# pashtari/factorizer

Hardware: AMD Instinct MI355X
Metric: volumes/sec fwd+bwd, Swin Factorizer 128^3 (higher is better)
Workload: dtype f32

## Files before the change

### factorizer_amd/_native.py

```python
from __future__ import annotations

import ctypes
import os
import threading

import torch

_HERE = os.path.dirname(os.path.abspath(__file__))
LIB_PATH = os.environ.get("FZ_LIB_PATH") or os.path.join(_HERE, "libfactorizer_hip.so")

FZ_OK = 0
FZ_E_UNSUPPORTED = -2
ABI_VERSION = 7
SOLVER_ID = {"mu": 0, "hals": 1, "cd": 2, "smu": 3}
STORE_F32, STORE_BF16 = 0, 1
PRODUCTS_DEFAULT, PRODUCTS_SPLIT_BF16, PRODUCTS_FP32_MFMA = 0, 1, 2
_products = threading.local()


def products() -> int:
    return getattr(_products, "value", PRODUCTS_DEFAULT)


class use_products:
# ... 132 lines not shown
                ("Di", _i), ("Hi", _i), ("Wi", _i), ("w", _vp), ("w_t", _i), ("ldw", _i), ("M", _i), ("K", _i),
                ("bias", _vp), ("ln", _i), ("ln_g", _vp), ("ln_b", _vp), ("ln_eps", _f), ("stats_out", _vp),
                ("bact", _i), ("bmul", _vp), ("bmul_kind", _i), ("eact", _i), ("res", _vp), ("emul", _vp), ("emul_kind", _i), ("y", _vp),
                ("Ncol", _i64), ("Ho", _i), ("Wo", _i), ("B", _i), ("loader", _i), ("epilogue", _i), ("lnb_x", _vp), ("lnb_stats", _vp), ("lnb_g", _vp),
                ("lnb_gadd", _vp), ("lnb_part", _vp), ("act_dtype", _i), ("products", _i), ("tune", _i)]


class MlpDesc(_c.Structure):
    _fields_ = [("mode", _i), ("inp", _vp), ("w1", _vp), ("w2", _vp), ("b1", _vp), ("b2", _vp), ("ln_g", _vp),
                ("ln_b", _vp), ("ln_eps", _f), ("stats", _vp), ("z1", _vp), ("gz1", _vp), ("x1", _vp), ("out", _vp),
                ("part", _vp), ("B", _i), ("C", _i), ("H", _i), ("V", _i64), ("act_dtype", _i), ("wpart", _vp),
                ("gw1", _vp), ("gb1", _vp), ("gw2", _vp), ("gb2", _vp), ("gln", _vp), ("glp", _vp), ("products", _i),
                ("pre_in", _vp), ("pre_w", _vp), ("pre_b", _vp), ("pre_res", _vp), ("pre_out", _vp),
                ("post_w", _vp), ("post_b", _vp), ("post_out", _vp), ("post_m", _i)]


class MlpDropout(_c.Structure):
    _fields_ = [("m0", _vp), ("m1", _vp), ("m2", _vp), ("s0", _f), ("s1", _f), ("s2", _f)]


class BlockPrologue(_c.Structure):
    _fields_ = [("ln_g", _vp), ("ln_b", _vp), ("ln_eps", _f), ("w", _vp), ("t", _vp), ("stats", _vp)]


class GemmDwDesc(_c.Structure):
    _fields_ = [("g", _vp), ("q", _vp), ("w", _vp), ("ln", _i), ("stats", _vp), ("ln_g", _vp), ("ln_b", _vp), ("gadd", _vp),
                ("y", _vp), ("gln", _vp), ("wpart", _vp), ("gw", _vp), ("gb", _vp), ("B", _i), ("C", _i), ("V", _i64),
                ("act_dtype", _i), ("ldgw", _i), ("ldw", _i), ("drop_m", _vp), ("drop_s", _f)]


class WgradDesc(_c.Structure):
    _fields_ = [("p", _vp), ("M", _i), ("pmul", _vp), ("pmul_kind", _i), ("q", _vp * 4), ("nsrc", _i),
                ("src_mode", _i), ("c0", _i), ("Cin", _i), ("K", _i), ("Vq", _i64), ("D", _i), ("H", _i),
                ("W", _i), ("N", _i64), ("Ho", _i), ("Wo", _i), ("stats", _vp), ("qact", _i), ("ln_g", _vp),
                ("ln_b", _vp), ("gw", _vp), ("gbias", _vp), ("accumulate", _i), ("B", _i), ("loader", _i),
                ("act_dtype", _i), ("products", _i)]


class VolGeom(_c.Structure):
    _fields_ = [("nd", _i), ("size", _i * 3), ("start", _i * 3), ("end", _i * 3), ("pad", _i * 3), ("out", _i * 3)]


class RespaceGeom(_c.Structure):
    _fields_ = [("nd", _i), ("src_size", _i * 3), ("src_axis", _i * 3), ("flip", _i * 3), ("res_size", _i * 3), ("pad", _i * 3),
                ("out", _i * 3), ("orig_size", _i * 3), ("box_start", _i * 3), ("scale", _c.c_double * 3),
                ("inv_scale", _c.c_double * 3)]


_SIGS.update({
    "fz_gcorr_supported": ([_i] * 5, _i),
    "fz_gcorr": ([_vp] * 5 + [_i] * 11 + [_f, _vp], _i),
    "fz_gcorr_wgrad_workspace_bytes": ([_i] * 10, _i64),
    "fz_gcorr_wgrad": ([_vp] * 4 + [_i] * 11 + [_vp], _i),
    "fz_gcorr_act": ([_vp] * 5 + [_i] * 11 + [_f, _i, _vp], _i),
    "fz_gcorr_wgrad_act": ([_vp] * 4 + [_i] * 12 + [_vp], _i),
    "fz_gcorr_mu_bwd": ([_vp] * 8 + [_i] * 11 + [_f, _i, _vp], _i),
    "fz_gnmf_supported": ([_i, _i64, _i, _i, _i], _i),
    "fz_gnmf_workspace_bytes": ([_i64, _i, _i64, _i, _i, _i], _i64),
    "fz_gnmf_launches": ([_i, _i, _i], _i),
    "fz_gnmf_fwd": ([_vp] * 6 + [_i64, _i, _i64, _i, _i, _i, _f, _vp, _vp], _i),
    "fz_gnmf_bwd": ([_vp] * 7 + [_i64, _i, _i64, _i, _i, _i, _i, _f, _vp, _vp], _i),
    "fz_nmf_cf_supported": ([_i] * 11, _i),
    "fz_nmf_cf_fwd": ([_vp] * 4 + [_i] * 5 + [_c.POINTER(_i)] + [_i] * 5 + [_f, _i, _vp], _i),
    "fz_nmf_cf_bwd": ([_vp] * 5 + [_i] * 5 + [_c.POINTER(_i)] + [_i] * 7 + [_f, _i, _vp], _i),
    "fz_nmf_cf_factors_supported": ([_i] * 12 + [_c.POINTER(_i)], _i),
    "fz_nmf_cf_fwd_store_factors": ([_vp] * 5 + [_i] * 5 + [_c.POINTER(_i)] + [_i] * 3 + [_f, _i, _vp], _i),
    "fz_nmf_cf_fwd_from_factors": ([_vp] * 6 + [_i] * 5 + [_c.POINTER(_i)] * 2 + [_i] * 4 + [_f, _i, _vp], _i),
    "fz_nmf_cf_bwd_factors_supported": ([_i] * 14 + [_c.POINTER(_i)], _i),
    "fz_nmf_cf_bwd_store_factors": ([_vp] * 5 + [_i] * 5 + [_c.POINTER(_i)] + [_i] * 3 + [_f, _i, _vp], _i),
    "fz_nmf_cf_bwd_from_factors": ([_vp] * 6 + [_i] * 5 + [_c.POINTER(_i)] * 2 + [_i] * 3 + [_f, _i, _vp], _i),
    "fz_nmf_pcf_supported": ([_i] * 11, _i),
    "fz_nmf_pcf_fwd": ([_vp] * 4 + [_i] * 8 + [_c.POINTER(_i)] + [_i] * 5 + [_f, _i, _vp], _i),
    "fz_nmf_pcf_bwd": ([_vp] * 5 + [_i] * 8 + [_c.POINTER(_i)] + [_i] * 7 + [_f, _i, _vp], _i),
    "fz_nmf_pcf_bwd_prefers_separate": ([_i] * 4, _i),
    "fz_act_add": ([_vp, _vp, _i64, _i, _vp], _i),
    "fz_mlp_pre_supported": ([_i, _i, _i64, _i], _i),
    "fz_mlp_drop_supported": ([_i, _i, _i64, _i], _i),
    "fz_mlp_chain_drop": ([_c.POINTER(MlpDesc), _c.POINTER(MlpDropout), _vp], _i),
    "fz_conv3_prologue_supported": ([_i] * 4, _i),
    "fz_conv3_fwd2": ([_vp] * 4 + [_i] * 8 + [_c.POINTER(BlockPrologue), _vp], _i),
    "fz_upcat2": ([_vp, _vp, _vp, _i, _vp, _vp, _vp] + [_i] * 7 + [_c.POINTER(BlockPrologue), _vp], _i),
    "fz_gemm": ([_c.POINTER(GemmDesc), _vp], _i),
    "fz_gemm_bx_enable": ([_i], _i),
    "fz_gemm_lnbwd_partials": ([_c.POINTER(GemmDesc)], _i64),
    "fz_reduce_rows": ([_vp, _i64, _i, _vp, _vp, _vp], _i),
    "fz_adamw_step": ([_vp, _vp, _vp, _vp, _i64, _f, _f, _f, _f, _f, _i, _f, _vp], _i),
    "fz_sw_gather": ([_vp, _vp] + [_i] * 10 + [_vp], _i),
    "fz_sw_accumulate": ([_vp] * 6 + [_f] + [_i] * 10 + [_vp], _i),
    "fz_sw_finalize": ([_vp, _vp, _i, _i64, _vp], _i),
    "fz_sw_gather2": ([_vp, _vp] + [_i] * 11 + [_vp], _i),
    "fz_sw_accumulate2": ([_vp] * 6 + [_f] + [_i] * 11 + [_vp], _i),
    "fz_sw_finalize2": ([_vp, _vp, _vp, _i, _i64, _i, _vp], _i),
    "fz_mlp_supported": ([_i, _i, _i64], _i),
    "fz_mlp_partials": ([_i, _i64], _i64),
    "fz_mlp_wgrad_rows": ([_i, _i64], _i),
    "fz_gemm_dw_rows": ([_i, _i64], _i),
    "fz_gemm_dw_workspace_bytes": ([_i, _i64], _i64),
    "fz_gemm_dw": ([_c.POINTER(GemmDwDesc), _vp], _i),
    "fz_mlp_wgrad_workspace_bytes": ([_i, _i64], _i64),
    "fz_mlp_chain": ([_c.POINTER(MlpDesc), _vp], _i),
    "fz_head_bwd_rows": ([], _i),
    "fz_head_bwd_workspace_bytes": ([], _i64),
    "fz_head_bwd": ([_vp, _vp, _vp, _vp, _vp, _i, _i, _i, _i64, _i, _vp], _i),
    "fz_head_fwd": ([_vp, _vp, _vp, _vp, _i, _i, _i, _i64, _i, _vp], _i),
    "fz_upcat_supported": ([_i] * 5, _i),
    "fz_upcat_compose": ([_vp, _vp, _i, _vp, _vp, _vp, _vp, _vp, _i, _i, _i, _vp], _i),
    "fz_upcat_wgrads": ([_vp, _vp, _vp, _i, _vp, _vp, _vp, _vp, _i, _vp, _i, _i, _i, _vp], _i),
    "fz_upcat": ([_vp, _vp, _vp, _i, _vp, _vp, _vp] + [_i] * 7 + [_vp], _i),
    "fz_upcat_bwd_supported": ([_i] * 6, _i),
    "fz_upcat_bwd_workspace_bytes": ([_i] * 4, _i64),
    "fz_upcat_bwd": ([_vp, _vp, _vp, _vp, _i, _vp, _vp, _vp, _vp, _vp, _i, _vp, _vp] + [_i] * 7 + [_vp], _i),
    "fz_wgrad": ([_c.POINTER(WgradDesc), _vp, _vp], _i),
    "fz_wgrad_group": ([_c.POINTER(_c.POINTER(WgradDesc)), _c.POINTER(_vp), _i, _vp], _i),
    "fz_wgrad_workspace_bytes": ([_c.POINTER(WgradDesc)], _i64),
    "fz_conv3_fwd": ([_vp] * 4 + [_i] * 8 + [_vp], _i),
    "fz_conv3_wgrad_chunks": ([_i] * 4, _i),
    "fz_conv3_wgrad_partials": ([_vp] * 4 + [_i] * 8 + [_vp], _i),
    "fz_chunk_reduce": ([_vp, _i, _i64, _vp, _i, _vp], _i),
    "fz_chunk_reduce_ld": ([_vp, _i, _i64, _i64, _vp, _i, _vp], _i),
    "fz_finish_defer": ([_i], _i),
    "fz_finish_pending": ([], _i),
    "fz_finish_flush": ([_vp], _i),
    "fz_finish_flush_all": ([_vp], _i),
    "fz_dice_bce_chunks": ([_i64], _i),
    "fz_dice_bce_sums": ([_vp, _vp, _vp, _i, _i64, _vp], _i),
    "fz_dice_bce_grad": ([_vp, _vp, _vp, _vp, _i, _i64, _f, _f, _vp, _vp], _i),
    "fz_dice_ce_sums": ([_vp, _vp, _vp, _i, _i, _i64, _vp], _i),
    "fz_dice_ce_grad": ([_vp, _vp, _vp, _vp, _i, _i, _i64, _f, _f, _vp, _vp], _i),
    "fz_dice_ce_finish": ([_vp, _i, _i, _i64, _f, _vp, _vp, _vp], _i),
    "fz_rowsum_chunks": ([_i64], _i),
    "fz_rowsum": ([_vp, _vp, _vp, _i, _i, _i64, _i, _vp], _i),
    "fz_ln_fwd": ([_vp] * 5 + [_i, _i, _i64, _f, _i, _vp], _i),
    "fz_ln_bwd": ([_vp] * 8 + [_i, _i, _i64, _i, _vp], _i),
    "fz_ln_bwd_workspace_bytes": ([_i], _i64),
    "fz_ln_bwd_workspace_bytes2": ([_i, _i, _i64], _i64),
    "fz_dropout_bits_words": ([_i, _i, _i64], _i64),
    "fz_dropout_keep_bits": ([_vp, _i, _i, _i, _i64, _f, _vp, _vp], _i),
    "fz_dropout_apply": ([_i, _vp, _f, _vp, _vp, _vp, _i, _i, _i64, _i, _vp], _i),
    "fz_seg_counts_chunks": ([_i64], _i),
    "fz_seg_counts_workspace_bytes": ([_i, _i64], _i64),
    "fz_seg_counts": ([_vp, _i, _vp, _i, _f, _vp, _vp, _vp, _i, _i64, _vp], _i),
    "fz_mask_edges": ([_vp, _vp, _vp, _i, _i, _i, _i, _i, _vp], _i),
    "fz_edge_min_dist2_splits": ([_i64, _i64], _i),
    "fz_edge_min_dist2_workspace_bytes": ([_i64, _i64], _i64),
    "fz_edge_min_dist2": ([_vp, _i64, _vp, _i64, _f, _f, _f, _vp, _vp, _vp], _i),
    "fz_aug_record_floats": ([], _i),
    "fz_aug_resample": ([_vp, _vp, _i, _i, _vp, _vp, _i, _vp, _vp, _vp] + [_i] * 6 + [_vp], _i),
    "fz_aug_smooth": ([_vp, _vp, _i, _i, _vp, _vp] + [_i] * 6 + [_vp], _i),
    "fz_aug_noise_field": ([_vp, _vp, _i, _i, _i64, _vp], _i),
    "fz_aug_source_words": ([], _i),
    "fz_aug_crop_resample": ([_vp, _vp, _i, _i, _vp, _i, _vp, _vp, _vp] + [_i] * 6 + [_vp], _i),
    "fz_vol_kind_ok": ([_i, _i], _i),
    "fz_vol_bbox": ([_vp, _i, _i, _i, _i, _i, _i, _vp, _vp], _i),
    "fz_vol_workspace_bytes": ([_i, _c.POINTER(VolGeom)], _i64),
    "fz_vol_stats": ([_vp, _i, _i, _c.POINTER(VolGeom), _i, _i, _vp, _vp], _i),
    "fz_vol_write": ([_vp, _i, _vp, _i, _i, _vp, _i, _i, _c.POINTER(_i), _c.POINTER(_i), _i, _vp, _c.POINTER(VolGeom), _i, _i,
                      _vp, _vp, _vp, _vp], _i),
    "fz_vol_restore": ([_c.POINTER(_vp), _i, _i, _i, _c.POINTER(VolGeom), _f, _c.POINTER(_c.c_ubyte), _vp, _vp], _i),
    "fz_vol_respace": ([_vp, _i, _vp, _i, _vp, _i, _vp, _c.POINTER(RespaceGeom), _i, _vp], _i),
    "fz_vol_unspace": ([_c.POINTER(_vp), _i, _i, _i, _c.POINTER(RespaceGeom), _i, _i, _f, _vp, _vp], _i),
})
SEG_F32, SEG_BF16, SEG_U8 = 0, 1, 2
VOL_F32, VOL_BF16, VOL_U8, VOL_I16 = 0, 1, 2, 3
VOL_IMAGE_IN, VOL_IMAGE_OUT, VOL_LABEL_IN, VOL_LOGITS = 0, 1, 2, 3
RESPACE_BILINEAR, RESPACE_NEAREST = 0, 1
DROP_RES, DROP_GELU, DROP_GELU_BWD = 0, 1, 2
# ... 1 lines not shown
```

### factorizer_amd/build.py

```python
from __future__ import annotations

import concurrent.futures as cf
import os
import shutil
import subprocess
import sys

HERE = os.path.dirname(os.path.abspath(__file__))
CSRC = os.path.join(HERE, "csrc")
OBJ = os.path.join(HERE, "csrc", "build")
LIB = os.path.join(HERE, "libfactorizer_hip.so")
ARCH = "gfx950"
FLAGS = ["--offload-arch=" + ARCH, "-O3", "-std=c++17", "-fPIC", "-fno-gpu-rdc", "-Wno-comment",
         "-ffp-contract=fast"]
_SLP_ON = {"gemm_bx.hip"}


def flags_of(src: str) -> list:
    return FLAGS if src in _SLP_ON else [*FLAGS, "-fno-slp-vectorize"]


def _hipcc() -> str:
    exe = shutil.which("hipcc") or "/opt/rocm/bin/hipcc"
    if not os.path.exists(exe):
        raise RuntimeError("hipcc not found: cannot build libfactorizer_hip.so")
    return exe


def sources():
    return sorted(f for f in os.listdir(CSRC) if f.endswith(".hip"))


def _newest(suffixes) -> float:
    m = 0.0
    for root in (CSRC, os.path.join(os.path.dirname(HERE), "include")):
        for f in os.listdir(root):
            if f.endswith(suffixes):
                m = max(m, os.path.getmtime(os.path.join(root, f)))
    return m


def _stale_flags() -> bool:
    for src in sources():
        stamp = os.path.join(OBJ, src[:-4] + ".o.flags")
        if not os.path.exists(stamp) or open(stamp).read() != " ".join(flags_of(src)):
            return True
    return False


def needs_build() -> bool:
    return not os.path.exists(LIB) or os.path.getmtime(LIB) < _newest((".h", ".inc", ".hip")) or _stale_flags()


def _compile(src: str) -> str:
    obj = os.path.join(OBJ, src[:-4] + ".o")
    flags = flags_of(src)
    stamp, want = obj + ".flags", " ".join(flags)
    fresh = os.path.exists(stamp) and open(stamp).read() == want
    if fresh and os.path.exists(obj) and os.path.getmtime(obj) >= max(os.path.getmtime(os.path.join(CSRC, src)), _newest((".h", ".inc"))):
        return obj
    cmd = [_hipcc(), *flags, "-c", os.path.join(CSRC, src), "-o", obj]
    r = subprocess.run(cmd, capture_output=True, text=True)
    if r.returncode != 0:
        raise RuntimeError(f"hipcc failed on {src}:\n{r.stderr[-4000:]}")
    with open(stamp, "w") as f:
        f.write(want)
    return obj


def build(force: bool = False, verbose: bool = True, jobs: int | None = None) -> str:
    if not force and not needs_build():
        return LIB
    os.makedirs(OBJ, exist_ok=True)
    srcs = sources()
    jobs = jobs or min(len(srcs), int(os.environ.get("MAX_JOBS") or 0) or min(os.cpu_count() or 4, 16))
    if verbose:
        print(f"[factorizer_amd] hipcc {ARCH}: {len(srcs)} translation units, {jobs} jobs", flush=True)
    with cf.ThreadPoolExecutor(jobs) as ex:
        objs = list(ex.map(_compile, srcs))
    tmp = LIB + ".tmp"
    r = subprocess.run([_hipcc(), "--offload-arch=" + ARCH, "-shared", "-fPIC", "-o", tmp, *objs],
                       capture_output=True, text=True)
    if r.returncode != 0:
        raise RuntimeError("link failed:\n" + r.stderr[-4000:])
    os.replace(tmp, LIB)
    if verbose:
        print(f"[factorizer_amd] built {LIB}", flush=True)
    return LIB


if __name__ == "__main__":
    build(force="--force" in sys.argv)
```

### factorizer_amd/csrc/gemm_bx.h

```cpp
#pragma once
#include "gemm_common.h"

namespace fz {

typedef __bf16 bx8 __attribute__((ext_vector_type(8)));
typedef __bf16 bx2 __attribute__((ext_vector_type(2)));
typedef float fx2 __attribute__((ext_vector_type(2)));

enum { BXPRO_NONE = 0, BXPRO_LN = 1, BXPRO_GELU = 2, BXPRO_BMUL = 3 };

template <int NT>
__device__ __forceinline__ void bx_split(const float (&x)[8], bx8 (&t)[NT]) {
#pragma unroll
  for (int i = 0; i < 8; i += 2) {
    fx2 v = {x[i], x[i + 1]};
    const bx2 a = __builtin_convertvector(v, bx2);
    t[0][i] = a[0]; t[0][i + 1] = a[1];
    if constexpr (NT >= 2) {
      v = v - __builtin_convertvector(a, fx2);
      const bx2 b = __builtin_convertvector(v, bx2);
      t[1][i] = b[0]; t[1][i + 1] = b[1];
      if constexpr (NT >= 3) {
        v = v - __builtin_convertvector(b, fx2);
        const bx2 c = __builtin_convertvector(v, bx2);
// ... 111 lines not shown
      constexpr int RBT = NACC == 4 ? 4 : (NACC == 2 ? 8 : 16);
#pragma unroll
      for (int r0 = 0; r0 < 16; r0 += RBT) {
      float ev[RBT][NACC], rv[RBT][NACC];
      if (p.emul != nullptr) {
#pragma unroll
        for (int rr = 0; rr < RBT; ++rr) uload<NACC>(p.emul + (urow + ((r0 + rr) & 3) + 8 * ((r0 + rr) >> 2)) * p.Ncol, yoff, ev[rr]);
      }
      if (p.res != nullptr) {
#pragma unroll
        for (int rr = 0; rr < RBT; ++rr) uload<NACC>(p.res + (urow + ((r0 + rr) & 3) + 8 * ((r0 + rr) >> 2)) * p.Ncol, yoff, rv[rr]);
      }
#pragma unroll
      for (int rr = 0; rr < RBT; ++rr) {
        const int r = r0 + rr;
        const int rl = (r & 3) + 8 * (r >> 2) + 4 * h;
        float add = sBias[mb * 32 + rl];
        float v[NACC];
        if (LN) {
          const float sw = sW[mb * 32 + rl];
          add += tW[mb * 32 + rl];
#pragma unroll
          for (int q = 0; q < NACC; ++q) v[q] = rstd[q] * (acc[mb][q][r] - mu_d[q] * sw) + add;
        } else {
#pragma unroll
          for (int q = 0; q < NACC; ++q) v[q] = acc[mb][q][r] + add;
        }
        if (p.eact) {
#pragma unroll
          for (int q = 0; q < NACC; ++q) v[q] = act_f(p.eact, v[q]);
        }
        if (p.emul != nullptr) {
#pragma unroll
          for (int q = 0; q < NACC; ++q) v[q] *= act_grad_f(p.emul_kind, ev[rr][q]);
        }
        if (p.res != nullptr) {
#pragma unroll
          for (int q = 0; q < NACC; ++q) v[q] += rv[rr][q];
        }
        AT* yp = reinterpret_cast<AT*>(reinterpret_cast<char*>(p.y + (urow + (r & 3) + 8 * (r >> 2)) * p.Ncol) + yoff);
        vstore<NACC>(yp, v);
      }
      }
    }
  } else {
    const int Wf = 2 * p.Wo, Hf = 2 * p.Ho;
    const int64_t Vf = 8 * p.Ncol;
    const int Mo = p.M >> 3;
    const int wo = (int)(col_off % p.Wo);
    const int64_t t2 = col_off / p.Wo;
    const int ho = (int)(t2 % p.Ho);
    const int dz = (int)(t2 / p.Ho);
    const unsigned foff = (unsigned)((((int64_t)(2 * dz + h) * Hf + 2 * ho) * Wf + 2 * wo) * ES);
#pragma unroll
    for (int mb = 0; mb < MB; ++mb) {
      const int64_t uo = (int64_t)b * Mo + ((m0 + mb * 32) >> 3);
      float rv[8][2 * NACC];
      if (p.res != nullptr) {
#pragma unroll
        for (int rp = 0; rp < 8; ++rp)
          uload<2 * NACC>(p.res + (uo + (rp >> 1)) * Vf + (int64_t)(rp & 1) * Wf, foff, rv[rp]);
      }
#pragma unroll
      for (int rp = 0; rp < 8; ++rp) {
        const int r0 = 2 * rp;
        const float bs = sBias[mb * 32 + 8 * (rp >> 1)];
        float v[2 * NACC];
#pragma unroll
        for (int q = 0; q < NACC; ++q) { v[2 * q] = acc[mb][q][r0] + bs; v[2 * q + 1] = acc[mb][q][r0 + 1] + bs; }
        if (p.res != nullptr) {
#pragma unroll
          for (int i = 0; i < 2 * NACC; ++i) v[i] += rv[rp][i];
        }
        AT* yp = reinterpret_cast<AT*>(reinterpret_cast<char*>(p.y + (uo + (rp >> 1)) * Vf + (int64_t)(rp & 1) * Wf) + foff);
        vstore<2 * NACC>(yp, v);
      }
    }
  }
}

template <typename AT>
int gemm_bxk_launch(const GemmArgsT<AT>& a, int loader, int epilogue, int pro, int nacc, int mb, fz_stream_t stream);

}
```

### factorizer_amd/csrc/gemm_bx.hip

```cpp
#include "gemm_bx.h"

namespace fz {

template <int MB, int NACC, int LOADER, int EPI, int PRO, int RD, bool WT, typename AT>
__global__ __launch_bounds__(256, 2) void gemm_bx_kernel(GemmArgsT<AT> p) {
  constexpr int NTA = BxTerms<AT>::A, NTB = bx_terms_b<AT>(PRO);
  constexpr int TN = 32 * NACC;
  constexpr bool S2D = LOADER == LOAD_S2D;
  static_assert(!S2D || NACC == 2, "space-to-depth loader: two coarse voxels per lane");
  constexpr int NL = S2D ? 4 : NACC;
  constexpr int SPG = S2D ? 4 : 8;
  constexpr int ES = (int)sizeof(AT);
  constexpr bool LN = PRO == BXPRO_LN, GATE = PRO == BXPRO_BMUL;
  constexpr int CH = 4;
  static_assert(CH % RD == 0, "ring slots must be static inside a chunk");
  constexpr int kItemHalfs = 8;
  constexpr int kBufItems = CH * MB * NTA * 64;
  constexpr int IPT = CH * MB * 64 / 256;
  __shared__ __attribute__((aligned(16))) __bf16 As[2 * kBufItems * kItemHalfs];
  __shared__ float sW[32 * MB];
  __shared__ float tW[32 * MB];
  __shared__ float sBias[32 * MB];
  __shared__ float sRed[LN ? 2 * 256 : 1];

// ... 211 lines not shown
  for (int e = 0; e < NACC; ++e) { mu_d[e] = 0.f; rstd[e] = 1.f; }
  if (LN) {
    sRed[threadIdx.x] = sWp;
    sRed[256 + threadIdx.x] = tWp;
    __syncthreads();
    if (threadIdx.x < 32 * MB) {
      const int mb = threadIdx.x >> 5, i = threadIdx.x & 31;
      float a = 0.f, c = 0.f;
      for (int w = mb; w < 4; w += MB)
        for (int hh = 0; hh < 2; ++hh) { a += sRed[64 * w + 32 * hh + i]; c += sRed[256 + 64 * w + 32 * hh + i]; }
      sW[threadIdx.x] = a;
      tW[threadIdx.x] = c;
    }
#pragma unroll
    for (int e = 0; e < NACC; ++e) {
      const float t1 = s1[e] + __shfl_xor(s1[e], 32, 64);
      const float t2 = s2[e] + __shfl_xor(s2[e], 32, 64);
      const float inv = 1.0f / (float)p.Cin;
      const float md = t1 * inv;
      float var = t2 * inv - md * md;
      var = var > 0.f ? var : 0.f;
      mu_d[e] = md;
      rstd[e] = 1.0f / sqrtf(var + p.ln_eps);
    }
    if (p.stats_out != nullptr && by == 0 && h == 0 && col_ok) {
      float mean[NACC];
#pragma unroll
      for (int e = 0; e < NACC; ++e) mean[e] = shift[e] + mu_d[e];
      float* so = p.stats_out + (int64_t)b * 2 * p.Vin;
      vstore<NACC>(so + col_off, mean);
      vstore<NACC>(so + p.Vin + col_off, rstd);
    }
    __syncthreads();
  }
  if (!col_ok) return;
  bx_epilogue<MB, NACC, EPI, S2D, LN, AT>(p, acc, b, m0, n0, j, h, col_off, sBias, sW, tW, rstd, mu_d);
}

template <typename AT>
bool gemm_bx_ok(const GemmArgsT<AT>& a, int loader, int epilogue, int pro, int nacc) {
  if (a.K % 32 != 0 || a.M % 32 != 0) return false;
  if (loader == LOAD_PLAIN && (a.c0 % 16 != 0 || a.Cin != a.K)) return false;
  if (loader == LOAD_S2D && (8 * a.Cin != a.K || pro != BXPRO_NONE || epilogue != EPI_PLAIN || (a.Wo & 1))) return false;
  if (epilogue == EPI_D2S && (pro != BXPRO_NONE || (nacc >= 2 && (a.Wo % nacc) != 0))) return false;
  if (a.Ncol % nacc != 0 || a.Vin % nacc != 0) return false;
  if (!a.w_t && ((a.ldw & 3) != 0 || (reinterpret_cast<uintptr_t>(a.w) & 15) != 0)) return false;
  if (pro == BXPRO_LN && ((reinterpret_cast<uintptr_t>(a.ln_g) & 15) != 0 || (reinterpret_cast<uintptr_t>(a.ln_b) & 15) != 0)) return false;
  const int64_t es = (int64_t)sizeof(AT);
  if ((8 * a.Vin + a.Vin) * es >= ((int64_t)1 << 31)) return false;
  if (((int64_t)a.M * a.ldw + 8 * a.ldw) * 4 >= ((int64_t)1 << 31)) return false;
  if ((4 * a.Ncol + a.Ncol) * es * 8 >= ((int64_t)1 << 31)) return false;
  return true;
}

template <typename AT>
int gemm_bx_launch(const GemmArgsT<AT>& a0, int loader, int epilogue, int pro, fz_stream_t stream) {
  GemmArgsT<AT> a = a0;
  hipStream_t st = (hipStream_t)stream;
  const int mblocks = (a.M + 31) / 32;
  int nacc, mb;
  {
    int ks = (a.Ncol * a.B <= 4096 || (a.Ncol * a.B <= 8192 && a.K >= 512)) ? 1 : 0;
    int kn = 2, km = mblocks >= 2 ? 2 : 1;
    auto wgs = [&](int na, int mbb) { return ((a.Ncol + 32 * na - 1) / (32 * na)) * a.B * ((mblocks + mbb - 1) / mbb); };
    if (wgs(kn, km) < 512 && km == 2) km = 1;
    if (wgs(kn, km) < 512 && loader != LOAD_S2D) kn = 1;
    if (a.tune >= 100) {
      ks = a.tune / 100 == 2;
      if (ks) { kn = (a.tune / 10) % 10; km = a.tune % 10; if (km > mblocks) km = 1; if (loader == LOAD_S2D) kn = 2; if (kn < 1 || kn > 2) kn = 2; if (km < 1 || km > 2) km = 1; }
    }
    if (ks) {
      const int rc = gemm_bxk_launch<AT>(a, loader, epilogue, pro, kn, km, stream);
      if (rc != FZ_E_UNSUPPORTED) return rc;
    }
  }
  if (loader == LOAD_S2D) {
    nacc = 2;
    mb = mblocks >= 2 ? 2 : 1;
  } else {
    nacc = 4; mb = mblocks >= 2 ? 2 : 1;
    auto wgs = [&](int na, int mbb) { return ((a.Ncol + 128 * na - 1) / (128 * na)) * a.B * ((mblocks + mbb - 1) / mbb); };
    if (wgs(nacc, mb) < 512) nacc = 2;
    if (wgs(nacc, mb) < 512 && mb == 2) mb = 1;
    if (a.tune / 100 == 1) { nacc = (a.tune / 10) % 10; mb = a.tune % 10; if (mb > mblocks || mb < 1) mb = 1; }
    if (nacc != 2 && nacc != 4) nacc = 2;
    if (pro == BXPRO_LN || pro == BXPRO_BMUL) nacc = 2;
  }
  if (mblocks % mb != 0) mb = 1;
  if (!gemm_bx_ok(a, loader, epilogue, pro, nacc)) return FZ_E_UNSUPPORTED;
  const int TN = 32 * nacc;
  const int64_t tiles = (a.Ncol + TN * 4 - 1) / (TN * 4);
  const int ygr = mblocks / mb;
  a.ygroups = (ygr > 1 && ygr <= 8 && tiles * a.B >= 64) ? ygr : 0;
  a.xtiles = (int)(tiles * a.B);
  dim3 grid((unsigned)(tiles * a.B), (unsigned)ygr), block(256);
  if (a.ygroups > 1) grid = dim3((unsigned)(((tiles * a.B + 7) / 8) * 8 * ygr), 1);
  const bool wt = a.w_t != 0;
#define FZ_BX(MBv, NAv, L, E, PR, RDv)                                                                           \
  do {                                                                                                           \
    if (wt) hipLaunchKernelGGL((gemm_bx_kernel<MBv, NAv, L, E, PR, RDv, true, AT>), grid, block, 0, st, a);      \
    else hipLaunchKernelGGL((gemm_bx_kernel<MBv, NAv, L, E, PR, RDv, false, AT>), grid, block, 0, st, a);        \
  } while (0)
#define FZ_BX_TILES(L, E, PR)                                                                                    \
  do {                                                                                                           \
    if (nacc == 4) { if (mb == 2) FZ_BX(2, 4, L, E, PR, 1); else FZ_BX(1, 4, L, E, PR, 2); }                      \
    else { if (mb == 2) FZ_BX(2, 2, L, E, PR, 4); else FZ_BX(1, 2, L, E, PR, 4); }                                \
  } while (0)
#define FZ_BX_TILES2(L, E, PR, RD2)                                                                              \
  do {                                                                                                           \
    if (mb == 2) FZ_BX(2, 2, L, E, PR, RD2); else FZ_BX(1, 2, L, E, PR, 4);                                       \
  } while (0)
  if (loader == LOAD_S2D) {
    if (mb == 2) FZ_BX(2, 2, LOAD_S2D, EPI_PLAIN, BXPRO_NONE, 4); else FZ_BX(1, 2, LOAD_S2D, EPI_PLAIN, BXPRO_NONE, 4);
  } else if (epilogue == EPI_D2S) FZ_BX_TILES(LOAD_PLAIN, EPI_D2S, BXPRO_NONE);
  else if (pro == BXPRO_LN) FZ_BX_TILES2(LOAD_PLAIN, EPI_PLAIN, BXPRO_LN, 4);
  else if (pro == BXPRO_GELU) FZ_BX_TILES(LOAD_PLAIN, EPI_PLAIN, BXPRO_GELU);
  else if (pro == BXPRO_BMUL) FZ_BX_TILES2(LOAD_PLAIN, EPI_PLAIN, BXPRO_BMUL, 2);
  else FZ_BX_TILES(LOAD_PLAIN, EPI_PLAIN, BXPRO_NONE);
  FZ_LAUNCH_CHECK();
  return FZ_OK;
}

template int gemm_bx_launch<float>(const GemmArgsT<float>&, int, int, int, fz_stream_t);
template int gemm_bx_launch<bf16>(const GemmArgsT<bf16>&, int, int, int, fz_stream_t);

}
```

### include/factorizer_hip.h

```cpp
#ifndef FACTORIZER_HIP_H
#define FACTORIZER_HIP_H

#include <stdint.h>

#ifdef __cplusplus
extern "C" {
#endif

#define FZ_OK 0
#define FZ_E_SHAPE (-1)
#define FZ_E_UNSUPPORTED (-2)
#define FZ_E_HIP (-3)
#define FZ_E_ARG (-4)

#define FZ_STORE_F32 0
#define FZ_STORE_BF16 1

#define FZ_SOLVER_MU 0
#define FZ_SOLVER_HALS 1
#define FZ_SOLVER_CD 2
#define FZ_SOLVER_SMU 3

typedef void* fz_stream_t;

// ... 54 lines not shown
                               void* out, int B, int C, int D, int H, int W, const int* shift, const int* prev_shift,
                               int divisor, int R, int T, int solver, float eps, int act_dtype, fz_stream_t stream);

int fz_nmf_cf_bwd_factors_supported(int C, int D, int H, int W, int d, int pd, int ph, int pw, int R, int T, int Tgrad,
                                    int solver, int relu_gate, int nshift, const int* shifts);
int fz_nmf_cf_bwd_store_factors(const void* t, const float* v0, const void* ga, float* gcfac, float* cofac, int B, int C,
                                int D, int H, int W, const int* shift, int nshift, int T, int Tgrad, float eps,
                                int act_dtype, fz_stream_t stream);
int fz_nmf_cf_bwd_from_factors(const void* t, const float* v0, const void* ga, const float* gcfac, const float* cofac,
                               void* gt, int B, int C, int D, int H, int W, const int* shift, const int* prev_shift,
                               int nshift, int T, int Tgrad, float eps, int act_dtype, fz_stream_t stream);

int fz_nmf_pcf_supported(int C, int D, int H, int W, int d, int pd, int ph, int pw, int R, int T, int Tgrad);
int fz_nmf_pcf_fwd(const void* t, const float* u0, const float* v0, void* out, int B, int C, int D, int H, int W,
                   int pd, int ph, int pw, const int* shift, int accumulate, int divisor, int R, int T, int solver,
                   float eps, int act_dtype, fz_stream_t stream);
int fz_nmf_pcf_bwd(const void* t, const float* u0, const float* v0, const void* ga, void* gt, int B, int C, int D,
                   int H, int W, int pd, int ph, int pw, const int* shift, int accumulate, int nshift, int relu_gate,
                   int R, int T, int Tgrad, int solver, float eps, int act_dtype, fz_stream_t stream);
int fz_nmf_pcf_bwd_prefers_separate(int pd, int ph, int pw, int act_dtype);
int fz_act_add(void* dst, const void* src, int64_t n, int act_dtype, fz_stream_t stream);

#define FZ_LOAD_PLAIN 0
#define FZ_LOAD_S2D 1
#define FZ_LOAD_K3 2
#define FZ_EPI_PLAIN 0
#define FZ_EPI_D2S 1
#define FZ_EPI_LNBWD 2
#define FZ_LOAD_S2D_2D 3
#define FZ_LOAD_K3_2D 4
#define FZ_EPI_D2S_2D 3
#define FZ_ACT_NONE 0
#define FZ_ACT_RELU 1
#define FZ_ACT_GELU 2

#define FZ_PRODUCTS_DEFAULT 0
#define FZ_PRODUCTS_SPLIT_BF16 1
#define FZ_PRODUCTS_FP32_MFMA 2

typedef struct fz_gemm_desc {
  const void* x[4];
  int nsrc;
  int src_mode;
  int c0;
  int Cin;
  int64_t Vin;
  int Di, Hi, Wi;
  const float* w;
  int w_t, ldw;
  int M, K;
  const float* bias;
  int ln;
  const float* ln_g;
  const float* ln_b;
  float ln_eps;
  float* stats_out;
  int bact;
  const void* bmul;
  int bmul_kind;
  int eact;
  const void* res;
  const void* emul;
  int emul_kind;
  void* y;
  int64_t Ncol;
  int Ho, Wo;
  int B;
  int loader, epilogue;
  const void* lnb_x;
  const float* lnb_stats;
  const float* lnb_g;
  const void* lnb_gadd;
  float* lnb_part;
  int act_dtype;
  int products;
  int tune;
} fz_gemm_desc;

int64_t fz_gemm_lnbwd_partials(const fz_gemm_desc* desc);
int fz_reduce_rows(const float* part, int64_t rows, int n, float* out, float* tmp, fz_stream_t stream);

int fz_gemm(const fz_gemm_desc* desc, fz_stream_t stream);
int fz_gemm_bx_enable(int on);

typedef struct fz_mlp_desc {
  int mode;
  const void* in;
  const float* w1;
  const float* w2;
  const float* b1;
  const float* b2;
  const float* ln_g;
  const float* ln_b;
  float ln_eps;
  float* stats;
  void* z1;
  void* gz1;
  const void* x1;
  void* out;
  float* part;
  int B, C, H;
  int64_t V;
  int act_dtype;
  void* wpart;
  float* gw1;
  float* gb1;
  float* gw2;
  float* gb2;
  float* gln;
  float* glp;
  int products;
  const void* pre_in;
  const float* pre_w;
  const float* pre_b;
  const void* pre_res;
  void* pre_out;
  const float* post_w;
  const float* post_b;
  void* post_out;
  int post_m;
} fz_mlp_desc;
typedef struct fz_mlp_dropout {
  const uint32_t* m0;
  const uint32_t* m1;
  const uint32_t* m2;
  float s0, s1, s2;
} fz_mlp_dropout;

typedef struct fz_gemm_dw_desc {
  const void* g;
  const void* q;
  const float* w;
  int ln;
  const float* stats;
  const float* ln_g;
  const float* ln_b;
  const void* gadd;
  void* y;
  float* gln;
  void* wpart;
  float* gw;
  float* gb;
  int B, C;
  int64_t V;
  int act_dtype;
  int ldgw;
  int ldw;
  const uint32_t* drop_m;
  float drop_s;
} fz_gemm_dw_desc;
int fz_gemm_dw_rows(int B, int64_t V);
int64_t fz_gemm_dw_workspace_bytes(int B, int64_t V);
int fz_gemm_dw(const fz_gemm_dw_desc* desc, fz_stream_t stream);

int fz_head_bwd_rows(void);
int64_t fz_head_bwd_workspace_bytes(void);
int fz_head_bwd(const void* gy, const void* x, const float* w, void* gx, float* part, int B, int M, int C, int64_t V,
                int act_dtype, fz_stream_t stream);
int fz_head_fwd(const void* x, const float* w, const float* bias, void* y, int B, int M, int C, int64_t V, int act_dtype,
                fz_stream_t stream);

int fz_upcat_compose(const float* w_t, const float* w_b, int ldb, const float* b_t, const float* b_ad, float* wc, float* wbt, float* bias,
                     int Cd, int O, int M, fz_stream_t stream);
int fz_upcat_wgrads(const float* gt, const float* w_t, const float* w_b, int ldb, const float* gb_ad, const float* b_t, float* gw_t,
                    float* gw_b, int ldg, float* gb_t, int Cd, int O, int M, fz_stream_t stream);
int fz_upcat_supported(int C, int Cd, int D, int H, int W);
// ... 216 lines not shown
```

Baseline: 134.4.

## Add persistent bf16-split GEMM kernel with weights resident in LDS

Adds a persistent-walker variant of the split-bf16 MFMA GEMM. Each workgroup converts and splits the whole weight slice into LDS once, then loops over many column tiles. Activation fetches for the next tile are prefetched across tile boundaries through a register ring. By default it only takes LN-prologue and depth-to-space epilogue GEMMs when there are enough tiles to fill the resident grid. This avoids re-splitting weights per tile and tail gaps between tiles, at the cost of large dynamic LDS, which limits occupancy, and more register pressure.

```diff
diff --git a/factorizer_amd/_native.py b/factorizer_amd/_native.py
--- a/factorizer_amd/_native.py
+++ b/factorizer_amd/_native.py
@@ -238,6 +238,8 @@
     "fz_upcat2": ([_vp, _vp, _vp, _i, _vp, _vp, _vp] + [_i] * 7 + [_c.POINTER(BlockPrologue), _vp], _i),
     "fz_gemm": ([_c.POINTER(GemmDesc), _vp], _i),
     "fz_gemm_bx_enable": ([_i], _i),
+    "fz_gemm_bxp_grid": ([_i], _i),
+    "fz_gemm_bxp_count": ([], _i64),
     "fz_gemm_lnbwd_partials": ([_c.POINTER(GemmDesc)], _i64),
     "fz_reduce_rows": ([_vp, _i64, _i, _vp, _vp, _vp], _i),
     "fz_adamw_step": ([_vp, _vp, _vp, _vp, _i64, _f, _f, _f, _f, _f, _i, _f, _vp], _i),
diff --git a/factorizer_amd/build.py b/factorizer_amd/build.py
--- a/factorizer_amd/build.py
+++ b/factorizer_amd/build.py
@@ -13,7 +13,7 @@
 ARCH = "gfx950"
 FLAGS = ["--offload-arch=" + ARCH, "-O3", "-std=c++17", "-fPIC", "-fno-gpu-rdc", "-Wno-comment",
          "-ffp-contract=fast"]
-_SLP_ON = {"gemm_bx.hip"}
+_SLP_ON = {"gemm_bx.hip", "gemm_bxp.hip"}
 
 
 def flags_of(src: str) -> list:
diff --git a/factorizer_amd/csrc/gemm_bx.h b/factorizer_amd/csrc/gemm_bx.h
--- a/factorizer_amd/csrc/gemm_bx.h
+++ b/factorizer_amd/csrc/gemm_bx.h
@@ -217,4 +217,7 @@
 template <typename AT>
 int gemm_bxk_launch(const GemmArgsT<AT>& a, int loader, int epilogue, int pro, int nacc, int mb, fz_stream_t stream);
 
-}
+template <typename AT>
+int gemm_bxp_launch(const GemmArgsT<AT>& a, int loader, int epilogue, int pro, int nacc, int mb, fz_stream_t stream);
+
+}
diff --git a/factorizer_amd/csrc/gemm_bx.hip b/factorizer_amd/csrc/gemm_bx.hip
--- a/factorizer_amd/csrc/gemm_bx.hip
+++ b/factorizer_amd/csrc/gemm_bx.hip
@@ -317,12 +317,16 @@
     auto wgs = [&](int na, int mbb) { return ((a.Ncol + 128 * na - 1) / (128 * na)) * a.B * ((mblocks + mbb - 1) / mbb); };
     if (wgs(nacc, mb) < 512) nacc = 2;
     if (wgs(nacc, mb) < 512 && mb == 2) mb = 1;
-    if (a.tune / 100 == 1) { nacc = (a.tune / 10) % 10; mb = a.tune % 10; if (mb > mblocks || mb < 1) mb = 1; }
+    if (a.tune / 100 == 1 || a.tune / 100 == 4) { nacc = (a.tune / 10) % 10; mb = a.tune % 10; if (mb > mblocks || mb < 1) mb = 1; }
     if (nacc != 2 && nacc != 4) nacc = 2;
     if (pro == BXPRO_LN || pro == BXPRO_BMUL) nacc = 2;
   }
   if (mblocks % mb != 0) mb = 1;
   if (!gemm_bx_ok(a, loader, epilogue, pro, nacc)) return FZ_E_UNSUPPORTED;
+  if (a.tune / 100 == 4 || a.tune < 100) {
+    const int rc = gemm_bxp_launch<AT>(a, loader, epilogue, pro, nacc, mb, stream);
+    if (rc != FZ_E_UNSUPPORTED) return rc;
+  }
   const int TN = 32 * nacc;
   const int64_t tiles = (a.Ncol + TN * 4 - 1) / (TN * 4);
   const int ygr = mblocks / mb;
diff --git a/factorizer_amd/csrc/gemm_bxp.hip b/factorizer_amd/csrc/gemm_bxp.hip
--- /dev/null
+++ b/factorizer_amd/csrc/gemm_bxp.hip
@@ -0,0 +1,381 @@
+#include <atomic>
+
+#include "gemm_bx.h"
+
+namespace fz {
+
+__host__ __device__ constexpr int bxp_image_bytes(int K, int mb, int nta) { return ((K + 63) / 64) * 64 * mb * nta * 64; }
+constexpr int kBxpImage2 = 72 * 1024;
+constexpr int kBxpImageMax = 96 * 1024;
+
+template <int MB, int NACC, int LOADER, int EPI, int PRO, int RD, typename AT>
+__global__ __launch_bounds__(256, 2) void gemm_bxp_kernel(GemmArgsT<AT> p, int ntiles, int nwalk) {
+  constexpr int NTA = BxTerms<AT>::A, NTB = bx_terms_b<AT>(PRO);
+  constexpr int TN = 32 * NACC;
+  constexpr bool S2D = LOADER == LOAD_S2D;
+  static_assert(!S2D || NACC == 2, "space-to-depth loader: two coarse voxels per lane");
+  constexpr int NL = S2D ? 4 : NACC;
+  constexpr int SPG = S2D ? 4 : 8;
+  constexpr int ES = (int)sizeof(AT);
+  constexpr bool LN = PRO == BXPRO_LN, GATE = PRO == BXPRO_BMUL;
+  constexpr int CH = 4;
+  static_assert(CH % RD == 0, "ring slots must be static inside a chunk");
+  constexpr int kItemHalfs = 8;
+  constexpr int IPT = CH * MB * 64 / 256;
+  extern __shared__ __attribute__((aligned(16))) __bf16 fz_lds_bxp[];
+  __bf16* As = fz_lds_bxp;
+  __shared__ float sW[32 * MB];
+  __shared__ float tW[32 * MB];
+  __shared__ float sBias[32 * MB];
+  __shared__ float sRed[LN ? 2 * 256 : 1];
+
+  const int lane = threadIdx.x & 63;
+  const int wave = __builtin_amdgcn_readfirstlane(threadIdx.x >> 6);
+  const int j = lane & 31, h = lane >> 5;
+  const int tiles_per_sample = (int)((p.Ncol + TN * 4 - 1) / (TN * 4));
+  const int xcd = blockIdx.x & 7, slot = blockIdx.x >> 3;
+  const int by = slot % p.ygroups;
+  const int walker = (slot / p.ygroups) * 8 + xcd;
+  if (walker >= nwalk || walker >= ntiles) return;
+  const int m0 = by * 32 * MB;
+  const int nG = p.K >> 4;
+  const int nGp = (nG + CH - 1) / CH * CH;
+
+  if (threadIdx.x < 32 * MB) {
+    const int m = m0 + threadIdx.x;
+    float bv = 0.f;
+    if (p.bias != nullptr) bv = (EPI == EPI_D2S) ? p.bias[m >> 3] : p.bias[m];
+    sBias[threadIdx.x] = bv;
+  }
+
+  struct Tile { int b; int n0; int col_off; bool col_ok; unsigned boff; };
+  auto decode = [&](int t) {
+    Tile c;
+    c.b = t / tiles_per_sample;
+    c.n0 = ((t - c.b * tiles_per_sample) * 4 + wave) * TN;
+    if (S2D) {
+      const int n = c.n0 + 2 * j;
+      c.col_ok = n < (int)p.Ncol;
+      const unsigned nn = c.col_ok ? (unsigned)n : 0u;
+      const unsigned wo = nn % (unsigned)p.Wo;
+      const unsigned t2 = nn / (unsigned)p.Wo;
+      const unsigned ho = t2 % (unsigned)p.Ho;
+      const unsigned dz = t2 / (unsigned)p.Ho;
+      c.col_off = (int)(((2 * dz) * (unsigned)p.Hi + 2 * ho) * (unsigned)p.Wi + 2 * wo);
+    } else {
+      c.col_off = c.n0 + NACC * j;
+      c.col_ok = c.col_off < (int)p.Ncol;
+    }
+    const int64_t coff = c.col_ok ? c.col_off : 0;
+    c.boff = (unsigned)(((int64_t)(S2D ? h : 8 * h) * p.Vin + coff) * ES);
+    return c;
+  };
+
+  struct Slot { float bv[SPG][GATE ? 2 * NL : NL]; };
+  auto fetch = [&](int gi, Slot& sl, int b, unsigned boff) {
+    const int g = gi >= nGp ? gi - nGp : (gi < nG ? gi : nG - 1);
+    if constexpr (!S2D) {
+      const int c16 = 16 * g;
+      const bool first = c16 < p.c0;
+      const AT* src = first ? p.x[0] : p.x[1];
+      const int cs = first ? p.c0 : p.Cin - p.c0;
+      const int ci = first ? c16 : c16 - p.c0;
+      const AT* ub = src + ((int64_t)b * cs + ci) * p.Vin;
+      const AT* ug = GATE ? p.bmul + ((int64_t)b * p.Cin + c16) * p.Vin : nullptr;
+#pragma unroll
+      for (int e = 0; e < 8; ++e) {
+        float a[NL];
+        uload<NL>(ub + (int64_t)e * p.Vin, boff, a);
+#pragma unroll
+        for (int i = 0; i < NL; ++i) sl.bv[e][i] = a[i];
+        if constexpr (GATE) {
+          float t[NL];
+          uload<NL>(ug + (int64_t)e * p.Vin, boff, t);
+#pragma unroll
+          for (int i = 0; i < NL; ++i) sl.bv[e][NL + i] = t[i];
+        }
+      }
+    } else {
+      const AT* ub = p.x[0] + ((int64_t)b * p.Cin + 2 * g) * p.Vin;
+#pragma unroll
+      for (int e = 0; e < 4; ++e) {
+        float a[NL];
+        uload<NL>(ub + (int64_t)(e >> 1) * p.Hi * p.Wi + (int64_t)(e & 1) * p.Wi, boff, a);
+#pragma unroll
+        for (int i = 0; i < NL; ++i) sl.bv[e][i] = a[i];
+      }
+    }
+  };
+  auto pivot = [&](const Tile& c, float (&shift)[NACC]) {
+    float pv[NL];
+    vload<NL>(p.x[0] + ((int64_t)c.b * p.c0) * p.Vin + (c.col_ok ? c.col_off : 0), pv);
+#pragma unroll
+    for (int e = 0; e < NACC; ++e) shift[e] = pv[e % NL];
+  };
+
+  auto fresh = [](int t) { asm volatile("" : "+s"(t)); return t; };
+  int tile = walker;
+  Tile cur = decode(tile);
+  int fb;
+  unsigned fboff;
+  Slot ring[RD];
+#pragma unroll
+  for (int i = 0; i < RD; ++i) fetch(i, ring[i], cur.b, cur.boff);
+  float shift[NACC];
+#pragma unroll
+  for (int e = 0; e < NACC; ++e) shift[e] = 0.f;
+  if (LN) pivot(cur, shift);
+
+  {
+    const int wl = threadIdx.x & 63;
+    const int wmb = (threadIdx.x >> 6) % MB;
+    const int wgl0 = (threadIdx.x >> 6) / MB;
+    const int wrow = m0 + wmb * 32 + (wl & 31);
+    const unsigned woff = p.w_t ? (unsigned)(((int64_t)8 * (wl >> 5) * p.ldw + wrow) * 4)
+                                : (unsigned)(((int64_t)wrow * p.ldw + 8 * (wl >> 5)) * 4);
+    const unsigned goff = (unsigned)(32 * (wl >> 5));
+    struct WRaw { float w[IPT][8]; float gm[LN ? IPT : 1][8]; float bt[LN ? IPT : 1][8]; };
+    float sWp = 0.f, tWp = 0.f;
+    auto issue = [&](int g0, WRaw& r) {
+#pragma unroll
+      for (int u = 0; u < IPT; ++u) {
+        int g = g0 + wgl0 + (4 / MB) * u;
+        g = g < nG ? g : nG - 1;
+        if (!p.w_t) {
+          uload<8>(p.w + 16 * g, woff, r.w[u]);
+        } else {
+          const float* uw = p.w + (int64_t)16 * g * p.ldw;
+#pragma unroll
+          for (int e = 0; e < 8; ++e) {
+            float t[1];
+            uload<1>(uw + (int64_t)e * p.ldw, woff, t);
+            r.w[u][e] = t[0];
+          }
+        }
+        if constexpr (LN) {
+          uload<8>(p.ln_g + 16 * g, goff, r.gm[u]);
+          uload<8>(p.ln_b + 16 * g, goff, r.bt[u]);
+        }
+      }
+    };
+    auto finish = [&](int g0, WRaw& r) {
+#pragma unroll
+      for (int u = 0; u < IPT; ++u) {
+        const float live = (g0 + wgl0 + (4 / MB) * u) < nG ? 1.0f : 0.0f;
+#pragma unroll
+        for (int e = 0; e < 8; ++e) r.w[u][e] *= live;
+        if constexpr (LN) {
+#pragma unroll
+          for (int e = 0; e < 8; ++e) {
+            tWp += r.w[u][e] * r.bt[u][e];
+            r.w[u][e] *= r.gm[u][e];
+            sWp += r.w[u][e];
+          }
+        }
+        const int gm = (threadIdx.x >> 6) + 4 * u;
+        bx8 t[NTA];
+        bx_split<NTA>(r.w[u], t);
+#pragma unroll
+        for (int i = 0; i < NTA; ++i)
+          *reinterpret_cast<bx8*>(&As[((g0 * MB + gm) * NTA + i) * 64 * kItemHalfs + wl * kItemHalfs]) = t[i];
+      }
+    };
+    WRaw ra, rb;
+    issue(0, ra);
+    for (int g0 = 0; g0 < nG; g0 += 2 * CH) {
+      issue(g0 + CH, rb);
+      finish(g0, ra);
+      if (g0 + CH < nG) {
+        issue(g0 + 2 * CH, ra);
+        finish(g0 + CH, rb);
+      }
+    }
+    if (LN) {
+      sRed[threadIdx.x] = sWp;
+      sRed[256 + threadIdx.x] = tWp;
+      __syncthreads();
+      if (threadIdx.x < 32 * MB) {
+        const int mb = threadIdx.x >> 5, i = threadIdx.x & 31;
+        float a = 0.f, c = 0.f;
+        for (int w = mb; w < 4; w += MB)
+          for (int hh = 0; hh < 2; ++hh) { a += sRed[64 * w + 32 * hh + i]; c += sRed[256 + 64 * w + 32 * hh + i]; }
+        sW[threadIdx.x] = a;
+        tW[threadIdx.x] = c;
+      }
+    }
+    __syncthreads();
+  }
+
+  for (; tile < ntiles; tile += nwalk) {
+    int tnext = tile + nwalk < ntiles ? tile + nwalk : tile;
+    {
+      const Tile c = decode(tile);
+      fb = c.b;
+      fboff = c.boff;
+    }
+
+    f32x16 acc[MB][NACC];
+#pragma unroll
+    for (int mb = 0; mb < MB; ++mb)
+#pragma unroll
+      for (int q = 0; q < NACC; ++q)
+#pragma unroll
+        for (int r = 0; r < 16; ++r) acc[mb][q][r] = 0.f;
+    float s1[NACC], s2[NACC];
+#pragma unroll
+    for (int e = 0; e < NACC; ++e) s1[e] = s2[e] = 0.f;
+
+    for (int g0 = 0; g0 < nG; g0 += CH) {
+      const __bf16* Ab = As + g0 * MB * NTA * 64 * kItemHalfs;
+#pragma unroll
+      for (int gl = 0; gl < CH; ++gl) {
+        Slot& sl = ring[gl % RD];
+        bx8 bop[NACC][NTB];
+#pragma unroll
+        for (int q = 0; q < NACC; ++q) {
+          float x[8];
+#pragma unroll
+          for (int e = 0; e < 8; ++e) {
+            float t;
+            if constexpr (S2D) {
+              t = sl.bv[e >> 1][2 * q + (e & 1)];
+            } else {
+              t = sl.bv[e][q];
+              if (GATE) t = sl.bv[e][NL + q] > 0.f ? t : 0.f;
+              if (LN) {
+                t -= shift[q];
+                const float tv = (g0 + gl < nG) ? t : 0.f;
+                s1[q] += tv;
+                s2[q] += tv * tv;
+              }
+              if (PRO == BXPRO_GELU) t = gelu_f(t);
+            }
+            x[e] = t;
+          }
+          bx_split<NTB>(x, bop[q]);
+        }
+        if (g0 + gl + RD == nGp) {
+          const Tile n = decode(fresh(tnext));
+          fb = n.b;
+          fboff = n.boff;
+        }
+        fetch(g0 + gl + RD, sl, fb, fboff);
+#pragma unroll
+        for (int mb = 0; mb < MB; ++mb) {
+          bx8 aop[NTA];
+#pragma unroll
+          for (int i = 0; i < NTA; ++i)
+            aop[i] = *reinterpret_cast<const bx8*>(&Ab[((gl * MB + mb) * NTA + i) * 64 * kItemHalfs + lane * kItemHalfs]);
+#pragma unroll
+          for (int q = 0; q < NACC; ++q) bx_mfma<NTA, NTB>(acc[mb][q], aop, bop[q]);
+        }
+      }
+    }
+
+    float mu_d[NACC], rstd[NACC];
+#pragma unroll
+    for (int e = 0; e < NACC; ++e) { mu_d[e] = 0.f; rstd[e] = 1.f; }
+    cur = decode(fresh(tile));
+    if (LN) {
+#pragma unroll
+      for (int e = 0; e < NACC; ++e) {
+        const float t1 = s1[e] + __shfl_xor(s1[e], 32, 64);
+        const float t2 = s2[e] + __shfl_xor(s2[e], 32, 64);
+        const float inv = 1.0f / (float)p.Cin;
+        const float md = t1 * inv;
+        float var = t2 * inv - md * md;
+        var = var > 0.f ? var : 0.f;
+        mu_d[e] = md;
+        rstd[e] = 1.0f / sqrtf(var + p.ln_eps);
+      }
+      if (p.stats_out != nullptr && by == 0 && h == 0 && cur.col_ok) {
+        float mean[NACC];
+#pragma unroll
+        for (int e = 0; e < NACC; ++e) mean[e] = shift[e] + mu_d[e];
+        float* so = p.stats_out + (int64_t)cur.b * 2 * p.Vin;
+        vstore<NACC>(so + cur.col_off, mean);
+        vstore<NACC>(so + p.Vin + cur.col_off, rstd);
+      }
+      pivot(decode(fresh(tnext)), shift);
+    }
+    if (cur.col_ok)
+      bx_epilogue<MB, NACC, EPI, S2D, LN, AT>(p, acc, cur.b, m0, (int64_t)cur.n0, j, h, (int64_t)cur.col_off, sBias, sW, tW, rstd, mu_d);
+  }
+}
+
+static int gemm_bxp_enabled() {
+  static const int on = []() { const char* e = getenv("FZ_GEMM_BXP"); return e ? (atoi(e) != 0) : 1; }();
+  return on;
+}
+static std::atomic<int> g_bxp_grid{0};
+static std::atomic<int64_t> g_bxp_count{0};
+
+template <typename AT>
+int gemm_bxp_launch(const GemmArgsT<AT>& a0, int loader, int epilogue, int pro, int nacc, int mb, fz_stream_t stream) {
+  GemmArgsT<AT> a = a0;
+  const bool forced = a.tune / 100 == 4;
+  if (!forced && !gemm_bxp_enabled()) return FZ_E_UNSUPPORTED;
+  if (a.K < 64) return FZ_E_UNSUPPORTED;
+  const int image = bxp_image_bytes(a.K, mb, BxTerms<AT>::A);
+  if (image > kBxpImageMax) return FZ_E_UNSUPPORTED;
+  const int mblocks = (a.M + 31) / 32;
+  const int ygr = mblocks / mb;
+  const int TN = 32 * nacc;
+  const int64_t tiles = (a.Ncol + TN * 4 - 1) / (TN * 4);
+  const int64_t ntiles = tiles * a.B;
+  if (ntiles >= ((int64_t)1 << 28) || a.Ncol >= ((int64_t)1 << 30)) return FZ_E_UNSUPPORTED;
+  const int cap = g_bxp_grid.load(std::memory_order_relaxed);
+  const int resident = image <= kBxpImage2 ? 512 : 256;
+  if (!forced) {
+    if (image > kBxpImage2) return FZ_E_UNSUPPORTED;
+    const int64_t g = cap > 0 && cap < resident ? cap : resident;
+    const int64_t onetile = ntiles * ygr;
+    bool on = false;
+    if (pro == BXPRO_LN) on = onetile >= 4 * g;
+    else if (epilogue == EPI_D2S) on = a.K >= 128 && onetile >= 2 * g;
+    if (!on) return FZ_E_UNSUPPORTED;
+  }
+  int nwalk = (cap > 0 ? cap : resident) / ygr;
+  if (nwalk < 1) nwalk = 1;
+  if (cap <= 0 && nwalk > ntiles) nwalk = (int)ntiles;
+  a.ygroups = ygr;
+  a.xtiles = (int)ntiles;
+  dim3 grid((unsigned)((nwalk + 7) / 8 * 8 * ygr)), block(256);
+  hipStream_t st = (hipStream_t)stream;
+#define FZ_BXP(MBv, NAv, L, E, PR, RDv)                                                                          \
+  do {                                                                                                           \
+    auto kern = gemm_bxp_kernel<MBv, NAv, L, E, PR, RDv, AT>;                                                    \
+    if (image > 64 * 1024)                                                                                       \
+      FZ_HIP_OK(hipFuncSetAttribute(reinterpret_cast<const void*>(kern), hipFuncAttributeMaxDynamicSharedMemorySize, image)); \
+    hipLaunchKernelGGL(kern, grid, block, image, st, a, (int)ntiles, nwalk);                                     \
+  } while (0)
+#define FZ_BXP_TILES(L, E, PR)                                                                                   \
+  do {                                                                                                           \
+    if (nacc == 4) { if (mb == 2) FZ_BXP(2, 4, L, E, PR, 1); else FZ_BXP(1, 4, L, E, PR, 2); }                    \
+    else { if (mb == 2) FZ_BXP(2, 2, L, E, PR, 4); else FZ_BXP(1, 2, L, E, PR, 4); }                              \
+  } while (0)
+#define FZ_BXP_TILES2(L, E, PR, RD2)                                                                             \
+  do {                                                                                                           \
+    if (mb == 2) FZ_BXP(2, 2, L, E, PR, RD2); else FZ_BXP(1, 2, L, E, PR, 4);                                     \
+  } while (0)
+  if (loader == LOAD_S2D) {
+    if (mb == 2) FZ_BXP(2, 2, LOAD_S2D, EPI_PLAIN, BXPRO_NONE, 4); else FZ_BXP(1, 2, LOAD_S2D, EPI_PLAIN, BXPRO_NONE, 4);
+  } else if (epilogue == EPI_D2S) FZ_BXP_TILES(LOAD_PLAIN, EPI_D2S, BXPRO_NONE);
+  else if (pro == BXPRO_LN) FZ_BXP_TILES2(LOAD_PLAIN, EPI_PLAIN, BXPRO_LN, 4);
+  else if (pro == BXPRO_GELU) FZ_BXP_TILES(LOAD_PLAIN, EPI_PLAIN, BXPRO_GELU);
+  else if (pro == BXPRO_BMUL) FZ_BXP_TILES2(LOAD_PLAIN, EPI_PLAIN, BXPRO_BMUL, 2);
+  else FZ_BXP_TILES(LOAD_PLAIN, EPI_PLAIN, BXPRO_NONE);
+  g_bxp_count.fetch_add(1, std::memory_order_relaxed);
+  FZ_LAUNCH_CHECK();
+  return FZ_OK;
+}
+
+template int gemm_bxp_launch<float>(const GemmArgsT<float>&, int, int, int, int, int, fz_stream_t);
+template int gemm_bxp_launch<bf16>(const GemmArgsT<bf16>&, int, int, int, int, int, fz_stream_t);
+
+}
+
+extern "C" int fz_gemm_bxp_grid(int workgroups) {
+  return fz::g_bxp_grid.exchange(workgroups > 0 ? workgroups : 0, std::memory_order_relaxed);
+}
+extern "C" int64_t fz_gemm_bxp_count(void) { return fz::g_bxp_count.load(std::memory_order_relaxed); }
diff --git a/include/factorizer_hip.h b/include/factorizer_hip.h
--- a/include/factorizer_hip.h
+++ b/include/factorizer_hip.h
@@ -160,6 +160,8 @@
 
 int fz_gemm(const fz_gemm_desc* desc, fz_stream_t stream);
 int fz_gemm_bx_enable(int on);
+int fz_gemm_bxp_grid(int workgroups);
+int64_t fz_gemm_bxp_count(void);
 
 typedef struct fz_mlp_desc {
   int mode;
```

Result: no change. 134.9, median of 6 (+0.4%).
